# mims-harvard/ProCyon

Measured on AMD Instinct MI355X. Metric: phenotype-gen tokens/sec (ProCyon-Full greedy generation, end to end), higher is better.
Workload: dtype bf16; 1 GPU; configs[1]: ProCyon-Full (ESM2-650M + Llama-3-8B geometry=full) bf16 batch=1, 1024-residue protein, 512-token prompt, 256-token greedy generation; parallelism=single GPU

## Files before the change

include/pcy.h:

```cpp
#ifndef PCY_H
#define PCY_H
#include <stddef.h>
#include <stdint.h>

#ifdef __cplusplus
extern "C" {
#endif

#define PCY_ABI_VERSION 13

typedef struct pcy_ctx pcy_ctx;

enum { PCY_EPI_STORE = 0, PCY_EPI_RESID = 1, PCY_EPI_GELU_ERF = 2, PCY_EPI_GELU_ESM = 3, PCY_EPI_SWIGLU = 4 };
enum { PCY_POOL_MEAN = 0, PCY_POOL_MEAN_CORRECTED = 1, PCY_POOL_MAX = 2 };

int pcy_abi_version(void);
unsigned long long pcy_debug_dispatch_count(int kind);
unsigned long long pcy_debug_extend_grouped_count(void);
const char* pcy_last_error(void);
int pcy_ctx_create(int device_id, void* stream, pcy_ctx** out);
void pcy_ctx_destroy(pcy_ctx* ctx);
int pcy_ctx_sync(pcy_ctx* ctx);
int pcy_timer_start(pcy_ctx* ctx);
int pcy_timer_stop(pcy_ctx* ctx, float* ms_out);
// ... 156 lines not shown
int pcy_llama_decode_gemm_mq(pcy_ctx*, const pcy_llama_desc*, const pcy_kv_cache*, const pcy_gen_state*, int B);
unsigned long long pcy_debug_attn_mq_count(void);
int pcy_attn_decode_split(pcy_ctx*, void* qkv, int ld, const pcy_kv_cache* kv, int layer, void* o, int ldo, const int32_t* pos,
                          const void* cos_t, const void* sin_t, const uint8_t* keep, int B, int H, int Hkv, int dh);
int pcy_attn_split_chunk_keys(int B, int rows_per_prefix, int H, int Hkv, int dh, int prefix_T);
int pcy_llama_decode_split(pcy_ctx*, const pcy_llama_desc*, const pcy_kv_cache*, const pcy_gen_state*, int B);
int pcy_llama_decode_gemm_split(pcy_ctx*, const pcy_llama_desc*, const pcy_kv_cache*, const pcy_gen_state*, int B);
unsigned long long pcy_debug_attn_split_count(void);
int pcy_gemv_w8(pcy_ctx*, const void* W8, const float* scale, const void* x, int ldx, const void* resid, void* y, int ldy, const void* rms_w,
                float rms_eps, int rms_cast, int N, int K, int B, int epi);
int pcy_llama_decode_w8(pcy_ctx*, const pcy_llama_desc*, const pcy_llama_layer_fp8* w8, const pcy_kv_cache*, const pcy_gen_state*, int B);
int pcy_llama_greedy_w8(pcy_ctx*, const pcy_llama_desc*, const pcy_llama_layer_fp8* w8, const pcy_kv_cache*, const pcy_gen_state*, int B,
                        int n_steps, int use_graph);
unsigned long long pcy_debug_decode_w8_count(void);
int pcy_greedy_pick(pcy_ctx*, const pcy_llama_desc*, const pcy_kv_cache*, const pcy_gen_state*, int B, int advance_pos);
typedef struct {
  int32_t* hist;
  int32_t* n_hist;
  int32_t* window;
  const int32_t* forced;
  int32_t* counters;
  int32_t* last;
  int32_t cap, W;
  int32_t ngram_max, ngram_min;
} pcy_look_state;
int pcy_look_draft(pcy_ctx*, const pcy_llama_desc*, const pcy_look_state*, const pcy_gen_state*, void* embeds_out);
int pcy_look_verify(pcy_ctx*, const pcy_llama_desc*, const pcy_look_state*, const pcy_gen_state*, const void* logits);
unsigned long long pcy_debug_look_count(int which);
int pcy_attn_window(pcy_ctx*, void* qkv, int ld, const pcy_kv_cache* kv, int layer, void* o, int ldo, const int32_t* pos, const void* cos_t,
                    const void* sin_t, int W, int H, int Hkv, int dh);
// ... 97 lines not shown
```

procyon_amd/_lib.py:

```python
from __future__ import annotations

import ctypes as C
import os

_HERE = os.path.dirname(os.path.abspath(__file__))
LIB_PATH = os.environ.get("PCY_LIB") or os.path.join(_HERE, "libpcy.so")

EPI_STORE, EPI_RESID, EPI_GELU_ERF, EPI_GELU_ESM, EPI_SWIGLU = range(5)
POOL_MEAN, POOL_MEAN_CORRECTED, POOL_MAX = range(3)
ABI_VERSION = 13
(DISPATCH_GEMM_128, DISPATCH_GEMM_64, DISPATCH_GEMM_BIG, DISPATCH_GEMM_BIG_PERSIST, DISPATCH_GEMM_SPLITK, DISPATCH_GEMM_FP8, DISPATCH_ATTN_FAST,
 DISPATCH_DEC_STEP_GQA, DISPATCH_GEMM_MID, DISPATCH_ESM_GRAPH, DISPATCH_DEC_STEP_MHA, DISPATCH_DEC_LAYER, DISPATCH_DEC_STEP_NB, DISPATCH_DEC_STEP_MB,
 DISPATCH_DEC_LOOP_STREAM, DISPATCH_DEC_LOOP_MFMA, DISPATCH_SHARED_PREFIX, DISPATCH_XENT, DISPATCH_EXTEND,
 DISPATCH_EXTEND_PACKED) = range(20)
DISPATCH_DECODE = dict(step_gqa=DISPATCH_DEC_STEP_GQA, step_mha=DISPATCH_DEC_STEP_MHA, layer=DISPATCH_DEC_LAYER, step_nb=DISPATCH_DEC_STEP_NB,
                       step_mb=DISPATCH_DEC_STEP_MB, loop_stream=DISPATCH_DEC_LOOP_STREAM, loop_mfma=DISPATCH_DEC_LOOP_MFMA)
ATTN_ROUTE_DH32, ATTN_ROUTE_DH64, ATTN_ROUTE_LDS128_1, ATTN_ROUTE_LDS128_2 = range(4)

vp = C.c_void_p
i32 = C.c_int32
ci = C.c_int


class MlpDesc(C.Structure):
# ... 146 lines not shown
    "pcy_llama_decode_gemm": (ci, [vp, C.POINTER(LlamaDesc), C.POINTER(KvCache), C.POINTER(GenState), ci]),
    "pcy_debug_decode_gemm_count": (C.c_ulonglong, []),
    "pcy_attn_decode_shared": (ci, [vp, vp, ci, C.POINTER(KvCache), ci, vp, ci, vp, vp, vp, vp, ci, ci, ci, ci]),
    "pcy_llama_decode_gemm_mq": (ci, [vp, C.POINTER(LlamaDesc), C.POINTER(KvCache), C.POINTER(GenState), ci]),
    "pcy_debug_attn_mq_count": (C.c_ulonglong, []),
    "pcy_attn_decode_split": (ci, [vp, vp, ci, C.POINTER(KvCache), ci, vp, ci, vp, vp, vp, vp, ci, ci, ci, ci]),
    "pcy_attn_split_chunk_keys": (ci, [ci, ci, ci, ci, ci, ci]),
    "pcy_llama_decode_split": (ci, [vp, C.POINTER(LlamaDesc), C.POINTER(KvCache), C.POINTER(GenState), ci]),
    "pcy_llama_decode_gemm_split": (ci, [vp, C.POINTER(LlamaDesc), C.POINTER(KvCache), C.POINTER(GenState), ci]),
    "pcy_debug_attn_split_count": (C.c_ulonglong, []),
    "pcy_gemv_w8": (ci, [vp, vp, vp, vp, ci, vp, vp, ci, vp, C.c_float, ci, ci, ci, ci, ci]),
    "pcy_llama_decode_w8": (ci, [vp, C.POINTER(LlamaDesc), C.POINTER(LlamaLayerFp8), C.POINTER(KvCache), C.POINTER(GenState), ci]),
    "pcy_llama_greedy_w8": (ci, [vp, C.POINTER(LlamaDesc), C.POINTER(LlamaLayerFp8), C.POINTER(KvCache), C.POINTER(GenState), ci, ci, ci]),
    "pcy_debug_decode_w8_count": (C.c_ulonglong, []),
    "pcy_greedy_pick": (ci, [vp, C.POINTER(LlamaDesc), C.POINTER(KvCache), C.POINTER(GenState), ci, ci]),
    "pcy_look_draft": (ci, [vp, C.POINTER(LlamaDesc), C.POINTER(LookState), C.POINTER(GenState), vp]),
    "pcy_look_verify": (ci, [vp, C.POINTER(LlamaDesc), C.POINTER(LookState), C.POINTER(GenState), vp]),
    "pcy_debug_look_count": (C.c_ulonglong, [ci]),
    "pcy_attn_window": (ci, [vp, vp, ci, C.POINTER(KvCache), ci, vp, ci, vp, vp, vp, ci, ci, ci, ci]),
    "pcy_attn_window_chunk": (ci, []),
    "pcy_llama_decode_window": (ci, [vp, C.POINTER(LlamaDesc), C.POINTER(KvCache), C.POINTER(GenState), vp, ci, vp]),
    "pcy_debug_decode_window_count": (C.c_ulonglong, []),
    "pcy_llama_greedy": (ci, [vp, C.POINTER(LlamaDesc), C.POINTER(KvCache), C.POINTER(GenState), ci, ci, ci]),
    "pcy_sample_pick": (ci, [vp, C.POINTER(LlamaDesc), C.POINTER(KvCache), C.POINTER(GenState), ci, ci, C.c_float, C.c_float, vp, vp]),
    "pcy_llama_sample": (ci, [vp, C.POINTER(LlamaDesc), C.POINTER(KvCache), C.POINTER(GenState), ci, ci, C.c_float, C.c_float, vp]),
    "pcy_beam_step": (ci, [vp, vp, ci, ci, ci, ci, C.c_float, C.POINTER(BeamState)]),
    "pcy_kv_reorder": (ci, [vp, C.POINTER(LlamaDesc), C.POINTER(KvCache), vp, ci, ci]),
    "pcy_kv_reorder_range": (ci, [vp, C.POINTER(LlamaDesc), C.POINTER(KvCache), vp, ci, ci, ci]),
    "pcy_llama_beam_steps": (ci, [vp, C.POINTER(LlamaDesc), C.POINTER(KvCache), C.POINTER(GenState), ci, ci, ci, C.c_float, C.POINTER(BeamState), vp, ci, ci]),
    "pcy_llama_beam_steps_split": (ci, [vp, C.POINTER(LlamaDesc), C.POINTER(KvCache), C.POINTER(GenState), ci, ci, ci, C.c_float, C.POINTER(BeamState), vp, ci, ci]),
# ... 33 lines not shown
```

procyon_amd/csrc/pcy_elem.hip:

```cpp
#include "pcy_internal.h"
#include "pcy_pick.h"

namespace {

constexpr int NT = 256;

__global__ __launch_bounds__(NT) void rmsnorm_kernel(const bf16_t* __restrict__ x, const bf16_t* __restrict__ w,
                                                     bf16_t* __restrict__ y, int d, float eps, int cast) {
  __shared__ float red[NT / 64];
  const bf16_t* xr = x + (size_t)blockIdx.x * d;
  bf16_t* yr = y + (size_t)blockIdx.x * d;
  float ss = 0.f;
  for (int k = threadIdx.x * 8; k < d; k += NT * 8) {
    const uint4 v = *reinterpret_cast<const uint4*>(xr + k);
    const uint32_t u[4] = {v.x, v.y, v.z, v.w};
#pragma unroll
    for (int j = 0; j < 4; ++j) { float a = lo_bf(u[j]), b = hi_bf(u[j]); ss += a * a + b * b; }
  }
  ss = block_sum<NT>(ss, red);
  const float rstd = rsqrtf(ss / (float)d + eps);
  for (int k = threadIdx.x * 8; k < d; k += NT * 8) {
    const uint4 v = *reinterpret_cast<const uint4*>(xr + k);
    const uint4 g = *reinterpret_cast<const uint4*>(w + k);
    const uint32_t u[4] = {v.x, v.y, v.z, v.w}, gg[4] = {g.x, g.y, g.z, g.w};
// ... 347 lines not shown
    const float v = wsum[((size_t)p * POOL_CH + ch) * d + c];
    if (mode == 2) a = fmaxf(a, v);
    else { a += v; n += wcnt[((size_t)p * POOL_CH + ch) * d + c]; }
  }
  out[(size_t)p * d + c] = (mode == 2) ? f2bf(a) : f2bf(rbf(a) / (float)n);
}


__global__ __launch_bounds__(PICK_NT) void pick_stage1_kernel(const bf16_t* __restrict__ logits, int V, PickPartial* __restrict__ part) {
  __shared__ float redv[PICK_NT / 64];
  __shared__ int redi[PICK_NT / 64];
  __shared__ float red[PICK_NT / 64];
  const int b = blockIdx.y, c = blockIdx.x;
  const int chunk = (V + PICK_NB - 1) / PICK_NB;
  const int lo = c * chunk, hi = (lo + chunk) < V ? (lo + chunk) : V;
  const bf16_t* lg = logits + (size_t)b * V;
  float best = -INFINITY;
  int bi = 0x7fffffff;
  for (int i = lo + threadIdx.x; i < hi; i += PICK_NT) {
    const float v = bf2f(lg[i]);
    if (v > best || (v == best && i < bi)) { best = v; bi = i; }
  }
#pragma unroll
  for (int o = 32; o > 0; o >>= 1) {
    const float ov = __shfl_xor(best, o, 64);
    const int oi = __shfl_xor(bi, o, 64);
    if (ov > best || (ov == best && oi < bi)) { best = ov; bi = oi; }
  }
  const int w = threadIdx.x >> 6;
  if ((threadIdx.x & 63) == 0) { redv[w] = best; redi[w] = bi; }
  __syncthreads();
  best = redv[0]; bi = redi[0];
  for (int i = 1; i < PICK_NT / 64; ++i)
    if (redv[i] > best || (redv[i] == best && redi[i] < bi)) { best = redv[i]; bi = redi[i]; }
  float se = 0.f;
  for (int i = lo + threadIdx.x; i < hi; i += PICK_NT) se += expf(bf2f(lg[i]) - best);
  se = block_sum<PICK_NT>(se, red);
  if (threadIdx.x == 0) part[b * PICK_NB + c] = PickPartial{best, bi, best > -INFINITY ? se : 0.f, 0};
}

__global__ __launch_bounds__(256) void pick_stage2_kernel(const bf16_t* __restrict__ logits, int V, const PickPartial* __restrict__ part,
                                                          int32_t* __restrict__ next_tok, int32_t* __restrict__ tokens_out, int max_steps,
                                                          float* __restrict__ logprob, int32_t* __restrict__ step_dev, int32_t* __restrict__ pos_dev,
                                                          int advance_pos, int B) {
  const int l = threadIdx.x & 63;
  const int step = *step_dev;
  for (int b = threadIdx.x >> 6; b < B; b += 4) {
    float best, se;
    int bi;
    pick_merge_row(part[b * PICK_NB + l], best, bi, se);
    if (l == 0) {
      const float lsm = pick_logprob(logits + (size_t)b * V, bi, best, se);
      logprob[b] += lsm;
      next_tok[b] = bi;
      tokens_out[(size_t)b * max_steps + step] = bi;
    }
  }
  __syncthreads();
  if (threadIdx.x == 0) { if (advance_pos) *pos_dev += 1; *step_dev = step + 1; }
}

constexpr int SMP_NT = 1024;

__global__ __launch_bounds__(PICK_NT) void sample_stage1_kernel(const bf16_t* __restrict__ logits, int V, float temperature,
                                                                float4* __restrict__ part) {
  __shared__ float red[PICK_NT / 64];
  const int b = blockIdx.y, c = blockIdx.x;
  const int chunk = (V + PICK_NB - 1) / PICK_NB;
  const int lo = c * chunk, hi = (lo + chunk) < V ? (lo + chunk) : V;
  const bf16_t* lg = logits + (size_t)b * V;
  const bool scaled = temperature != 1.0f;
  float mr = -INFINITY, ms = -INFINITY;
  for (int i = lo + threadIdx.x; i < hi; i += PICK_NT) {
    const float v = bf2f(lg[i]);
// ... 863 lines not shown
  if (nprot <= 0) return;
  float* wsum = reinterpret_cast<float*>(ws);
  int* wcnt = reinterpret_cast<int*>(wsum + (size_t)nprot * POOL_CH * d);
  hipLaunchKernelGGL(pool_partial_kernel, dim3(nprot, (d + 511) / 512, POOL_CH), dim3(NT), 0, s, h, d, seg, rng, mode, wsum, wcnt);
  hipLaunchKernelGGL(pool_finish_kernel, dim3(nprot, (d + NT - 1) / NT), dim3(NT), 0, s, wsum, wcnt, d, mode, out);
}
void pcy_launch_pick_stage1(hipStream_t s, const bf16_t* logits, int rows, int V, void* partials) {
  if (rows > 0) hipLaunchKernelGGL(pick_stage1_kernel, dim3(PICK_NB, rows), dim3(PICK_NT), 0, s, logits, V, reinterpret_cast<PickPartial*>(partials));
}
void pcy_launch_greedy_pick(hipStream_t s, const bf16_t* logits, int B, int V, int32_t* next_tok, int32_t* tokens_out,
                            int max_steps, float* logprob, int32_t* pos_dev, int32_t* step_dev, int advance_pos, void* partials) {
  hipLaunchKernelGGL(pick_stage1_kernel, dim3(PICK_NB, B), dim3(PICK_NT), 0, s, logits, V, reinterpret_cast<PickPartial*>(partials));
  hipLaunchKernelGGL(pick_stage2_kernel, dim3(1), dim3(256), 0, s, logits, V, reinterpret_cast<const PickPartial*>(partials), next_tok,
                     tokens_out, max_steps, logprob, step_dev, pos_dev, advance_pos, B);
}
int pcy_sample_max_vocab() { return SMP_NT * SMP_KMAX; }
void pcy_launch_sample_step(hipStream_t s, const bf16_t* logits, int B, int V, float temperature, float nucleus_p, const float* uniforms,
                            unsigned* hist, bf16_t* probs_out, int32_t* next_tok, int32_t* tokens_out, int max_steps, float* logprob,
                            int32_t* pos_dev, int32_t* step_dev, int advance_pos, void* partials, bf16_t* pbits) {
  hipLaunchKernelGGL(sample_stage1_kernel, dim3(PICK_NB, B), dim3(PICK_NT), 0, s, logits, V, temperature, reinterpret_cast<float4*>(partials));
  hipLaunchKernelGGL(sample_probs_kernel, dim3(PICK_NB, B), dim3(PICK_NT), 0, s, logits, V, reinterpret_cast<const float4*>(partials), temperature,
                     nucleus_p > 0.f ? 1 : 0, hist, pbits);
  hipLaunchKernelGGL(sample_stage2_kernel, dim3(B), dim3(SMP_NT), 0, s, logits, V, reinterpret_cast<const float4*>(partials), temperature,
                     nucleus_p, uniforms, hist, probs_out, next_tok, tokens_out, max_steps, logprob, step_dev, B, pbits);
  hipLaunchKernelGGL(sample_advance_kernel, dim3(1), dim3(64), 0, s, pos_dev, step_dev, advance_pos);
}
void pcy_launch_copy_rows(hipStream_t s, const bf16_t* src, int lds_, bf16_t* dst, int ldd, const int32_t* rows, int nrows, int d) {
  if (nrows > 0) hipLaunchKernelGGL(copy_rows_kernel, dim3(nrows), dim3(NT), 0, s, src, lds_, dst, ldd, rows, d);
}
void pcy_launch_l2norm_rows(hipStream_t s, const bf16_t* x, bf16_t* y, int rows, int d, float eps) {
// ... 46 lines not shown
```

procyon_amd/csrc/pcy_engine.hip:

```cpp
#include <stdio.h>
#include <stdlib.h>
#include <stdarg.h>
#include <string.h>
#include <dlfcn.h>
#include <vector>

#include "../../include/pcy.h"
#include "pcy_internal.h"

namespace {

thread_local char g_err[512] = "";

int fail(int code, const char* fmt, ...) {
  va_list ap;
  va_start(ap, fmt);
  vsnprintf(g_err, sizeof(g_err), fmt, ap);
  va_end(ap);
  return code;
}

#define HIP_TRY(expr)                                                                       \
  do {                                                                                      \
    hipError_t e_ = (expr);                                                                 \
// ... 1 lines not shown
  } while (0)

inline size_t align_up(size_t v, size_t a) { return (v + a - 1) / a * a; }

inline bool kv_shared(const pcy_kv_cache* kv) { return kv->prefix_k != nullptr || kv->prefix_v != nullptr || kv->prefix_T != 0; }
inline int kv_cap(const pcy_kv_cache* kv) { return kv->Tmax + (kv_shared(kv) ? kv->prefix_T : 0); }
unsigned long long g_pcy_extend_grouped = 0;
unsigned long long g_pcy_look[2] = {0, 0};
unsigned long long g_pcy_decode_gemm = 0;
unsigned long long g_pcy_attn_mq = 0;
unsigned long long g_pcy_attn_split = 0;
unsigned long long g_pcy_decode_w8 = 0;
unsigned long long g_pcy_decode_window = 0;
unsigned long long g_pcy_f32_stream = 0;
unsigned long long g_pcy_f32_select[2] = {0, 0};

}

void pcy_set_error(const char* fmt, ...) {
  va_list ap;
  va_start(ap, fmt);
  vsnprintf(g_err, sizeof(g_err), fmt, ap);
  va_end(ap);
}

enum GraphKind {
  KIND_GREEDY = 0,
  KIND_DECODE = 1,
  KIND_BEAM = 2,
  KIND_GREEDY_W8 = 3,
// ... 42 lines not shown
  size_t mc_tags_words = 0;
  PcySwitches mc_tags_sw = {};
  uint64_t layers_fp = 0;
  PcyLayerWeightsDev* dev_layers = nullptr;
  uint32_t* nb_tags[9] = {};
  unsigned* nb_sync = nullptr;
  unsigned* mb_flags = nullptr;
  size_t mb_flags_words = 0;
  unsigned* mb_sync = nullptr;
  uint32_t* op_tags = nullptr;
  size_t op_tags_words = 0;
  unsigned* smp_hist = nullptr;
  int smp_hist_rows = 0;
  bf16_t* smp_pbits = nullptr;
  size_t smp_pbits_elems = 0;
  char* beam_ws = nullptr;
  size_t beam_ws_bytes = 0;

  struct GraphSlot { uint64_t key[16]; hipGraphExec_t exec; unsigned long long stamp; };
  static constexpr int N_GSLOTS = 8;
  GraphSlot gslots[N_GSLOTS] = {};
  unsigned long long gstamp = 0;
  void drop_gslots() {
    for (auto& g : gslots) {
      if (g.exec) hipGraphExecDestroy(g.exec);
      g = GraphSlot{};
    }
  }

  int reserve(size_t bytes) {
// ... 96 lines not shown
int ensure_sync_words(pcy_ctx* c) {
  if (!c->n_cu) {
    hipDeviceProp_t prop;
    HIP_TRY(hipGetDeviceProperties(&prop, c->device));
    c->n_cu = prop.multiProcessorCount;
  }
  if (!c->xwg_err) {
    HIP_TRY(hipHostMalloc(reinterpret_cast<void**>(&c->xwg_err), 64, hipHostMallocMapped | hipHostMallocCoherent));
    memset(c->xwg_err, 0, 64);
  }
  if (!c->ao_sync) {
    const size_t bytes = (size_t)(64 + 2 * AO_MAX_LAYERS * AO_FLAGS) * sizeof(unsigned);
    HIP_TRY(hipMalloc(reinterpret_cast<void**>(&c->ao_sync), bytes));
    HIP_TRY(hipMemset(c->ao_sync, 0, bytes));
  }
  return 0;
}
uint64_t fnv1a(uint64_t h, std::initializer_list<const void*> ptrs) {
  for (const void* p : ptrs) h = (h ^ (uint64_t)(uintptr_t)p) * 1099511628211ull;
  return h;
}
constexpr uint64_t FNV_BASIS = 1469598103934665603ull;
uint64_t layers_fingerprint(const pcy_llama_desc* m) {
  uint64_t h = fnv1a(FNV_BASIS, {m->layers});
  for (int l = 0; l < m->n_layers; ++l) {
    const pcy_llama_layer& L = m->layers[l];
    h = fnv1a(h, {L.ln1, L.wqkv, L.wo, L.ln2, L.wgu, L.wdown});
  }
  return h;
}
// ... 365 lines not shown
void enqueue_lm_head(const DecodeCx& cx, const DecodePlan& p, void* logits_out, int xn_ready, bool force_stream = false) {
  const pcy_llama_desc* m = cx.m;
  PcyGemvArgs h{};
  h.W = (const bf16_t*)m->lm_head; h.x = cx.x; h.y = (bf16_t*)logits_out; h.rms_w = (const bf16_t*)m->final_norm; h.rms_eps = m->rms_eps;
  h.rms_cast = m->rms_cast; h.N = m->vocab; h.K = m->d; h.B = cx.B; h.ldx = m->d; h.ldy = m->vocab; h.epi = EPI_STORE;
  if (p.batched_head && !(p.nb_on && cx.B <= 4)) {
    norm_if_needed(cx, true, m->final_norm, &xn_ready);
    h.x = cx.xn; h.rms_w = nullptr;
  } else {
    h.force_stream = p.nb_on || force_stream;
  }
  pcy_launch_gemv(cx.c->stream, h);
}

void enqueue_decode(pcy_ctx* c, const pcy_llama_desc* m, const pcy_kv_cache* kv, const pcy_gen_state* st, int B, const PcySwitches& sw, bool layers_only = false,
                    bool split = false) {
  hipStream_t s = c->stream;
  const int d = m->d, dh = m->head_dim;
  const DecodeCx cx = decode_cx(c, m, kv, st, B);
  DecodePlan p = plan_decode(c, m, kv, B, sw);
  if (split) { p.defer_qkv_finish = false; p.attn_o = false; }
  if (layers_only) {
    if (p.epoch_word) pcy_launch_bump(s, p.epoch_word);
    if (p.tag_word) pcy_launch_bump(s, p.tag_word);
  } else {
    pcy_launch_embed_tokens_dev(s, (const bf16_t*)m->embed, st->next_tok, cx.x, B, d, p.epoch_word, p.tag_word);
  }
  const size_t tag_stride = tag_words_per_layer(m);
  bool step_done = false;
  const bool try_layer = p.path == DEC_STEP_GQA || p.path == DEC_STEP_MHA || p.path == DEC_LAYERS;
  int xn_ready = 0;
  if (p.path == DEC_STEP_NB) {
    const PcyDecodeStepArgs sa = step_args(cx, c->nb_tags[B], pcy_decode_nb_tag_words(B), 2 * AO_FLAGS, pcy_decode_nb_line_words(B));
    step_done = pcy_launch_decode_step_nb(s, c->device, attn_args(cx, p, -1), block_args(cx, p.tag_word, mc_trace(sw)), mlp_args(cx, p.tag_word), sa, c->n_cu,
                                          c->ao_sync, B, sw.nb_ub);
    if (step_done) ++g_pcy_dispatch[PCY_DISPATCH_DEC_STEP_NB];
  } else if (p.path == DEC_STEP_GQA || p.path == DEC_STEP_MHA) {
    const PcyDecodeStepArgs sa = step_args(cx, c->mc_tags, tag_stride, AO_FLAGS, 32 * 256);
    step_done = pcy_launch_decode_step(s, attn_args(cx, p, -1), block_args(cx, p.tag_word, mc_trace(sw)), mlp_args(cx, p.tag_word), sa, c->n_cu,
                                       c->ao_sync);
// ... 37 lines not shown
    const int b = (int)(i / chunks), c = (int)(i % chunks);
    const bf16_t* src = logits + (size_t)b * V + c * 8;
    bf16_t* dst = all + (step * B + b) * ld + c * 8;
    if (vec && c * 8 + 8 <= V) {
      const uint32_t w0 = src[0] | ((uint32_t)src[1] << 16), w1 = src[2] | ((uint32_t)src[3] << 16);
      const uint32_t w2 = src[4] | ((uint32_t)src[5] << 16), w3 = src[6] | ((uint32_t)src[7] << 16);
      *reinterpret_cast<uint4*>(dst) = make_uint4(w0, w1, w2, w3);
    } else {
      for (int e = 0; e < 8 && c * 8 + e < V; ++e) dst[e] = src[e];
    }
  }
}
void enqueue_store_logits(hipStream_t s, const void* logits, void* all, int ld, const int32_t* step_dev, int B, int V) {
  if (all) hipLaunchKernelGGL(store_logits_kernel, dim3(B >= 8 ? 256 : 64), dim3(256), 0, s, (const bf16_t*)logits, (bf16_t*)all, step_dev, B, V, ld > 0 ? ld : V);
}
void enqueue_pick(pcy_ctx* c, const pcy_llama_desc* m, const pcy_gen_state* st, int B, int advance_pos, int Tmax) {
  enqueue_store_logits(c->stream, st->logits, st->logits_all, st->logits_all_ld, st->step, B, m->vocab);
  pcy_launch_greedy_pick(c->stream, (const bf16_t*)st->logits, B, m->vocab, st->next_tok, st->tokens_out, st->max_steps,
                         st->logprob, st->pos, st->step, advance_pos, carve_decode_ws(c->ws, m, B, Tmax).partials);
}

void enqueue_sample(pcy_ctx* c, const pcy_llama_desc* m, const pcy_gen_state* st, int B, int advance_pos, int Tmax, float temperature,
                    float nucleus_p, const float* uniforms, bf16_t* probs_out) {
  hipStream_t s = c->stream;
  if (nucleus_p > 0.f) temperature = 1.0f;
  enqueue_store_logits(s, st->logits, st->logits_all, st->logits_all_ld, st->step, B, m->vocab);
  void* partials = carve_decode_ws(c->ws, m, B, Tmax).partials;
  pcy_launch_sample_step(s, (const bf16_t*)st->logits, B, m->vocab, temperature, nucleus_p, uniforms, c->smp_hist, probs_out, st->next_tok,
                         st->tokens_out, st->max_steps, st->logprob, st->pos, st->step, advance_pos, partials, c->smp_pbits);
}
int ensure_sample_state(pcy_ctx* c, int B, int V) {
  if ((size_t)B * V > c->smp_pbits_elems) {
    if (c->smp_pbits) { HIP_TRY(hipStreamSynchronize(c->stream)); HIP_TRY(hipFree(c->smp_pbits)); c->smp_pbits = nullptr; c->smp_pbits_elems = 0; }
    HIP_TRY(hipMalloc(reinterpret_cast<void**>(&c->smp_pbits), (size_t)B * V * 2));
// ... 98 lines not shown
}
void pcy_ctx_destroy(pcy_ctx* c) {
  if (!c) return;
  hipStreamSynchronize(c->stream);
  c->drop_graph();
  c->drop_gslots();
  if (c->ws) hipFree(c->ws);
  if (c->xwg_err) hipHostFree(c->xwg_err);
  if (c->ao_sync) hipFree(c->ao_sync);
  if (c->mc_tags) hipFree(c->mc_tags);
  if (c->dev_layers) hipFree(c->dev_layers);
  for (auto& t : c->nb_tags) if (t) hipFree(t);
  if (c->nb_sync) hipFree(c->nb_sync);
  if (c->mb_flags) hipFree(c->mb_flags);
  if (c->mb_sync) hipFree(c->mb_sync);
  if (c->op_tags) hipFree(c->op_tags);
  if (c->beam_ws) hipFree(c->beam_ws);
  if (c->smp_hist) hipFree(c->smp_hist);
  if (c->smp_pbits) hipFree(c->smp_pbits);
  if (c->ev0) hipEventDestroy(c->ev0);
  if (c->ev1) hipEventDestroy(c->ev1);
  if (c->cap_stream) hipStreamDestroy(c->cap_stream);
  delete c;
}
int pcy_ctx_sync(pcy_ctx* c) {
  HIP_TRY(hipStreamSynchronize(c->stream));
  return take_sticky_error(c);
}
int pcy_timer_start(pcy_ctx* c) { HIP_TRY(hipEventRecord(c->ev0, c->stream)); return 0; }
int pcy_timer_stop(pcy_ctx* c, float* ms) {
// ... 915 lines not shown
  if (int r = decode_prologue(c, m, kv, st, B, "pcy_llama_decode", step_ws_bytes, &sw)) return r;
  enqueue_decode(c, m, kv, st, B, sw);
  return check_launch("pcy_llama_decode");
}

int pcy_llama_decode_layers(pcy_ctx* c, const pcy_llama_desc* m, const pcy_kv_cache* kv, const pcy_gen_state* st, int B, int reps) {
  PCY_STICKY(c);
  PcySwitches sw;
  if (int r = decode_prologue(c, m, kv, st, B, "pcy_llama_decode_layers", step_ws_bytes, &sw)) return r;
  return run_steps(c, reps, false, "pcy_llama_decode_layers", DecodeGraphKey{}, [&] { enqueue_decode(c, m, kv, st, B, sw, true); });
}

int pcy_greedy_pick(pcy_ctx* c, const pcy_llama_desc* m, const pcy_kv_cache* kv, const pcy_gen_state* st, int B, int advance_pos) {
  PCY_STICKY(c);
  if (int r = c->reserve(decode_ws_bytes(m, B, kv_cap(kv)))) return r;
  enqueue_pick(c, m, st, B, advance_pos, kv_cap(kv));
  return check_launch("pcy_greedy_pick");
}

static int look_args(const char* what, const pcy_look_state* ls, const pcy_gen_state* st, PcyLookArgs* a) {
  if (!ls || !st) return fail(1, "%s: state missing", what);
  if (ls->W < 2 || ls->W > 32) return fail(1, "%s: W=%d outside [2, 32]", what, ls->W);
  if (ls->ngram_min < 1 || ls->ngram_max < ls->ngram_min || ls->ngram_max > 16)
    return fail(1, "%s: n-gram range [%d, %d] (1 <= min <= max <= 16)", what, ls->ngram_min, ls->ngram_max);
  if (ls->cap < 1 || !ls->hist || !ls->n_hist || !ls->window || !ls->counters || !ls->last) return fail(1, "%s: history / window / counters missing", what);
  if (!st->pos || !st->step || !st->next_tok || !st->tokens_out || !st->logprob || st->max_steps < 1) return fail(1, "%s: generation state incomplete", what);
  *a = PcyLookArgs{ls->hist, ls->n_hist, ls->window, ls->forced, ls->counters, ls->last, ls->cap, ls->W, ls->ngram_max, ls->ngram_min,
                   st->pos, st->step, st->next_tok, st->tokens_out, st->logprob, st->max_steps};
  return 0;
}
int pcy_look_draft(pcy_ctx* c, const pcy_llama_desc* m, const pcy_look_state* ls, const pcy_gen_state* st, void* embeds_out) {
// ... 12 lines not shown
  if (int r = look_args("pcy_look_verify", ls, st, &a)) return r;
  if (!logits) return fail(1, "pcy_look_verify: logits is NULL");
  if (int r = c->reserve(pcy_look_verify_ws_bytes(a.W))) return r;
  pcy_launch_look_verify(c->stream, a, (const bf16_t*)logits, m->vocab, (bf16_t*)st->logits_all, st->logits_all_ld, c->ws);
  ++g_pcy_look[1];
  return check_launch("pcy_look_verify");
}
unsigned long long pcy_debug_look_count(int which) { return (which == 0 || which == 1) ? g_pcy_look[which] : 0; }


int pcy_llama_greedy(pcy_ctx* c, const pcy_llama_desc* m, const pcy_kv_cache* kv, const pcy_gen_state* st, int B, int n_steps,
                     int use_graph) {
  PCY_STICKY(c);
  PcySwitches sw;
  if (int r = decode_prologue(c, m, kv, st, B, "pcy_llama_greedy", step_ws_bytes, &sw)) return r;
  DecodeGraphKey key;
  decode_graph_key(key, c, m, kv, st, B, KIND_GREEDY, sw);
  key_record(key, st);
  return run_steps(c, n_steps, use_graph != 0, "pcy_llama_greedy", key, [&] {
    enqueue_decode(c, m, kv, st, B, sw);
    enqueue_pick(c, m, st, B, 1, kv_cap(kv));
  });
}

int pcy_llama_decode_graph(pcy_ctx* c, const pcy_llama_desc* m, const pcy_kv_cache* kv, const pcy_gen_state* st, int B) {
  PCY_STICKY(c);
  PcySwitches sw;
  if (int r = decode_prologue(c, m, kv, st, B, "pcy_llama_decode_graph", step_ws_bytes, &sw)) return r;
  DecodeGraphKey key;
  decode_graph_key(key, c, m, kv, st, B, KIND_DECODE, sw);
  key_record(key, st);
  return run_steps(c, 1, true, "pcy_llama_decode_graph", key, [&] { enqueue_decode(c, m, kv, st, B, sw); });
}


static void enqueue_decode_gemm(pcy_ctx* c, const pcy_llama_desc* m, const pcy_kv_cache* kv, const pcy_gen_state* st, int B, bool mq, bool split = false) {
// ... 83 lines not shown
  if (pcy_gemv_w8_rows_per_pass(d) < 1 || pcy_gemv_w8_rows_per_pass(F) < 1 || pcy_gemv_w8_rows_per_pass(H * dh) < 1)
    return fail(1, "%s: a row of x (d, ffn or H*dh elements) does not fit in LDS", what);
  return c->reserve(decode_ws_bytes(m, B, kv_cap(kv)));
}
int pcy_llama_decode_w8(pcy_ctx* c, const pcy_llama_desc* m, const pcy_llama_layer_fp8* w8, const pcy_kv_cache* kv, const pcy_gen_state* st, int B) {
  PCY_STICKY(c);
  if (int r = decode_w8_check(c, m, w8, kv, st, B, "pcy_llama_decode_w8")) return r;
  enqueue_decode_w8(c, m, w8, kv, st, B);
  return check_launch("pcy_llama_decode_w8");
}
int pcy_llama_greedy_w8(pcy_ctx* c, const pcy_llama_desc* m, const pcy_llama_layer_fp8* w8, const pcy_kv_cache* kv, const pcy_gen_state* st, int B,
                        int n_steps, int use_graph) {
  PCY_STICKY(c);
  if (int r = decode_w8_check(c, m, w8, kv, st, B, "pcy_llama_greedy_w8")) return r;
  if (!st->step || !st->tokens_out || !st->logprob) return fail(1, "pcy_llama_greedy_w8: generation state incomplete");
  DecodeGraphKey key;
  key_base(key, KIND_GREEDY_W8, B, m, kv, st, c, layers_fingerprint(m));
  key.keep = st->keep; key.w8 = w8; key.w8_fp = w8_fingerprint(m, w8);
  key_record(key, st);
  return run_steps(c, n_steps, use_graph != 0, "pcy_llama_greedy_w8", key, [&] {
    enqueue_decode_w8(c, m, w8, kv, st, B);
    enqueue_pick(c, m, st, B, 1, kv_cap(kv));
  });
}
unsigned long long pcy_debug_decode_w8_count(void) { return g_pcy_decode_w8; }

struct F32StreamCx { float *x, *xn, *qkv, *ao, *act; };
static F32StreamCx f32_stream_carve(char* ws, const pcy_f32_llama_desc* m, int B) {
  Carver cv(ws);
  F32StreamCx cx;
  cx.x = cv.take<float>((size_t)B * m->d);
  cx.xn = cv.take<float>((size_t)B * m->d);
  cx.qkv = cv.take<float>((size_t)B * (m->n_heads + 2 * m->n_kv_heads) * m->head_dim);
  cx.ao = cv.take<float>((size_t)B * m->n_heads * m->head_dim);
  cx.act = cv.take<float>((size_t)B * m->ffn);
  return cx;
}
static size_t f32_stream_ws_bytes(const pcy_f32_llama_desc* m, int B) {
  const size_t f = (size_t)B * (2 * (size_t)m->d + (size_t)(2 * m->n_heads + 2 * m->n_kv_heads) * m->head_dim + (size_t)m->ffn) * sizeof(float);
  return f + 8 * 256;
// ... 412 lines not shown
```

procyon_amd/csrc/pcy_internal.h:

```cpp
#pragma once
#include "pcy_common.h"
#include "pcy_switch.h"

struct PcyGemvArgs {
  const bf16_t* W;
  const bf16_t* x;
  bf16_t* y;
  const bf16_t* bias;
  const bf16_t* resid;
  const bf16_t* rms_w;
  float rms_eps;
  int rms_cast;
  int N, K, B, ldx, ldy, epi;
  int plain_loads;
  float* splitk_ws; size_t splitk_ws_bytes;
  const bf16_t* next_rms_w; bf16_t* next_xn; int* fused_next;
  int* defer_finish;
  int force_stream;
  int force_mfma;
  int krot;
};
void pcy_launch_gemv(hipStream_t s, const PcyGemvArgs& a);

struct PcyGemvW8Args {
// ... 317 lines not shown
  unsigned* err;
  unsigned long long* trace;
  int abl;
};
size_t pcy_decode_mb_flag_words();
int pcy_decode_mb_ds(int B);
bool pcy_decode_mb_fits(int B, int Tmax);
bool pcy_launch_decode_step_mb(hipStream_t s, int device, const PcyMbArgs& a, int n_cu);

size_t pcy_pool_ws_bytes(int nprot, int d);
void pcy_launch_pool(hipStream_t s, const bf16_t* h, int d, const int32_t* seg, const int32_t* rng, int nprot,
                     int mode, bf16_t* out, void* ws);
void pcy_launch_greedy_pick(hipStream_t s, const bf16_t* logits, int B, int V, int32_t* next_tok, int32_t* tokens_out,
                            int max_steps, float* logprob, int32_t* pos_dev, int32_t* step_dev, int advance_pos,
                            void* partials );
void pcy_launch_pick_stage1(hipStream_t s, const bf16_t* logits, int rows, int V, void* partials);
struct PcyLookArgs {
  int32_t* hist; int32_t* n_hist; int32_t* window; const int32_t* forced; int32_t* counters; int32_t* last;
  int cap, W, gmax, gmin;
  int32_t* pos; int32_t* step; int32_t* next_tok; int32_t* tokens_out; float* logprob; int max_steps;
};
size_t pcy_look_verify_ws_bytes(int W);
void pcy_launch_look_draft(hipStream_t s, const PcyLookArgs& a, const bf16_t* embed, int V, int d, bf16_t* embeds_out );
void pcy_launch_look_verify(hipStream_t s, const PcyLookArgs& a, const bf16_t* logits , int V, bf16_t* logits_all, int logits_all_ld,
                            void* partials );
void pcy_launch_retrieval_dot_f32(hipStream_t s, const float* query, int Q, const void* targets, int targets_bf16, int N, int D, float eps, float* sims);
size_t pcy_retrieval_dot_smem(int D);
void pcy_launch_retrieval_rank_f32(hipStream_t s, const float* sims, int Q, int N, int k, int32_t* idx_out, float* score_out);
int pcy_sample_max_vocab();
void pcy_launch_sample_step(hipStream_t s, const bf16_t* logits, int B, int V, float temperature, float nucleus_p, const float* uniforms,
// ... 26 lines not shown
```

procyon_amd/csrc/pcy_pick.h:

```cpp
#pragma once
#include "pcy_common.h"

constexpr int PICK_NT = 256;
constexpr int PICK_NB = 64;
struct PickPartial { float mx; int idx; float se; int pad; };

__device__ __forceinline__ void pick_merge_row(const PickPartial pp, float& best, int& bi, float& se) {
  best = pp.mx;
  bi = pp.idx;
#pragma unroll
  for (int o = 32; o > 0; o >>= 1) {
    const float ov = __shfl_xor(best, o, 64);
    const int oi = __shfl_xor(bi, o, 64);
    if (ov > best || (ov == best && oi < bi)) { best = ov; bi = oi; }
  }
  se = pp.se * expf(pp.mx - best);
  se = wave_sum(se);
}
__device__ __forceinline__ float pick_logprob(const bf16_t* __restrict__ row_logits, int bi, float best, float se) {
  return rbf((bf2f(row_logits[bi]) - best) - logf(se));
}
```

procyon_amd/csrc/pcy_switch.h:

```cpp
#pragma once
#include <stdint.h>
#include <stdlib.h>
#include <string.h>
#include <type_traits>

#define PCY_SWITCH_NAMES(X)                                                                                                                \
  X(attn_o) X(mlp_chain) X(decode_layer) X(decode_step) X(attn_qkv_finish) X(finish_norm) X(fp8_fused_norm) X(prefill_post_qkv) X(gemv_lds) \
  X(gemv_mfma4) X(fa_vrow) X(gelu_fast) X(esm_graph) X(lds_prefetch) X(decode_nb) X(decode_nb_step) X(beam_graph) X(kv_permute)             \
  X(decode_mb_step) X(beam_prefill_once) X(beam_kv_suffix) X(beam_kv_shared)
enum PcySwitch {
#define X(n) PCY_SW_##n,
  PCY_SWITCH_NAMES(X)
#undef X
  PCY_SW_COUNT
};
static_assert(PCY_SW_COUNT <= 32, "PcySwitches::off_mask holds one bit per name");

inline bool pcy_list_has(const char* list, const char* name) {
  if (!list) return false;
  const size_t n = strlen(name);
  for (const char* p = list; (p = strstr(p, name)) != nullptr; p += n)
    if ((p == list || p[-1] == ',') && (p[n] == 0 || p[n] == ',')) return true;
  return false;
}
// ... 39 lines not shown
```

Baseline: 397.1 tokens/s.

## Fuse logits store, greedy pick, and next-token embedding into one last-block kernel

Replaces the three-kernel greedy pick tail (store logits, stage-1 partials, stage-2 merge, plus the next step's embed kernel) with a single kernel. Each block copies its slice of logits and computes its partial. An atomic ticket elects the last block, which merges all partials, writes the token and logprob, bumps the step and pos counters, and gathers the next token's embedding row into the decode input buffer. The goal is to cut per-token kernel launches and the serialization gaps between them in the 256-step decode loop. In exchange it relies on a ticket counter with release/acquire fences, and it moves the first embed kernel out of the captured step.

```diff
diff --git a/include/pcy.h b/include/pcy.h
--- a/include/pcy.h
+++ b/include/pcy.h
@@ -194,6 +194,7 @@
                         int n_steps, int use_graph);
 unsigned long long pcy_debug_decode_w8_count(void);
 int pcy_greedy_pick(pcy_ctx*, const pcy_llama_desc*, const pcy_kv_cache*, const pcy_gen_state*, int B, int advance_pos);
+unsigned long long pcy_debug_pick_tail_count(int which);
 typedef struct {
   int32_t* hist;
   int32_t* n_hist;
diff --git a/procyon_amd/_lib.py b/procyon_amd/_lib.py
--- a/procyon_amd/_lib.py
+++ b/procyon_amd/_lib.py
@@ -184,6 +184,7 @@
     "pcy_llama_greedy_w8": (ci, [vp, C.POINTER(LlamaDesc), C.POINTER(LlamaLayerFp8), C.POINTER(KvCache), C.POINTER(GenState), ci, ci, ci]),
     "pcy_debug_decode_w8_count": (C.c_ulonglong, []),
     "pcy_greedy_pick": (ci, [vp, C.POINTER(LlamaDesc), C.POINTER(KvCache), C.POINTER(GenState), ci, ci]),
+    "pcy_debug_pick_tail_count": (C.c_ulonglong, [ci]),
     "pcy_look_draft": (ci, [vp, C.POINTER(LlamaDesc), C.POINTER(LookState), C.POINTER(GenState), vp]),
     "pcy_look_verify": (ci, [vp, C.POINTER(LlamaDesc), C.POINTER(LookState), C.POINTER(GenState), vp]),
     "pcy_debug_look_count": (C.c_ulonglong, [ci]),
diff --git a/procyon_amd/csrc/pcy_elem.hip b/procyon_amd/csrc/pcy_elem.hip
--- a/procyon_amd/csrc/pcy_elem.hip
+++ b/procyon_amd/csrc/pcy_elem.hip
@@ -385,29 +385,8 @@
   const int b = blockIdx.y, c = blockIdx.x;
   const int chunk = (V + PICK_NB - 1) / PICK_NB;
   const int lo = c * chunk, hi = (lo + chunk) < V ? (lo + chunk) : V;
-  const bf16_t* lg = logits + (size_t)b * V;
-  float best = -INFINITY;
-  int bi = 0x7fffffff;
-  for (int i = lo + threadIdx.x; i < hi; i += PICK_NT) {
-    const float v = bf2f(lg[i]);
-    if (v > best || (v == best && i < bi)) { best = v; bi = i; }
-  }
-#pragma unroll
-  for (int o = 32; o > 0; o >>= 1) {
-    const float ov = __shfl_xor(best, o, 64);
-    const int oi = __shfl_xor(bi, o, 64);
-    if (ov > best || (ov == best && oi < bi)) { best = ov; bi = oi; }
-  }
-  const int w = threadIdx.x >> 6;
-  if ((threadIdx.x & 63) == 0) { redv[w] = best; redi[w] = bi; }
-  __syncthreads();
-  best = redv[0]; bi = redi[0];
-  for (int i = 1; i < PICK_NT / 64; ++i)
-    if (redv[i] > best || (redv[i] == best && redi[i] < bi)) { best = redv[i]; bi = redi[i]; }
-  float se = 0.f;
-  for (int i = lo + threadIdx.x; i < hi; i += PICK_NT) se += expf(bf2f(lg[i]) - best);
-  se = block_sum<PICK_NT>(se, red);
-  if (threadIdx.x == 0) part[b * PICK_NB + c] = PickPartial{best, bi, best > -INFINITY ? se : 0.f, 0};
+  const PickPartial pp = pick_chunk_partial(logits + (size_t)b * V, lo, hi, redv, redi, red);
+  if (threadIdx.x == 0) part[b * PICK_NB + c] = pp;
 }
 
 __global__ __launch_bounds__(256) void pick_stage2_kernel(const bf16_t* __restrict__ logits, int V, const PickPartial* __restrict__ part,
@@ -429,6 +408,87 @@
   }
   __syncthreads();
   if (threadIdx.x == 0) { if (advance_pos) *pos_dev += 1; *step_dev = step + 1; }
+}
+
+__global__ __launch_bounds__(PICK_NT) void pick_tail_kernel(PcyPickTailArgs a) {
+  __shared__ float redv[PICK_NT / 64];
+  __shared__ int redi[PICK_NT / 64];
+  __shared__ float red[PICK_NT / 64];
+  __shared__ int last_s;
+  __shared__ int tok_s[PICK_EMBED_ROWS];
+  const int b = blockIdx.y, c = blockIdx.x, V = a.V, B = gridDim.y;
+  const int chunk = (V + PICK_NB - 1) / PICK_NB;
+  const int lo = c * chunk, hi = (lo + chunk) < V ? (lo + chunk) : V;
+  const bf16_t* lg = a.logits + (size_t)b * V;
+  PickPartial* part = reinterpret_cast<PickPartial*>(a.partials);
+  const int step = *a.step_dev;
+  if (a.all) {
+    const bool vec = (a.ld % 8 == 0) && ((reinterpret_cast<uintptr_t>(a.all) & 15) == 0);
+    bf16_t* row = a.all + ((size_t)step * B + b) * a.ld;
+    for (int p = ((lo + 7) >> 3) + threadIdx.x; p * 8 < hi; p += PICK_NT) {
+      const bf16_t* src = lg + p * 8;
+      bf16_t* dst = row + p * 8;
+      if (vec && p * 8 + 8 <= V) {
+        const uint32_t w0 = src[0] | ((uint32_t)src[1] << 16), w1 = src[2] | ((uint32_t)src[3] << 16);
+        const uint32_t w2 = src[4] | ((uint32_t)src[5] << 16), w3 = src[6] | ((uint32_t)src[7] << 16);
+        *reinterpret_cast<uint4*>(dst) = make_uint4(w0, w1, w2, w3);
+      } else {
+        for (int e = 0; e < 8 && p * 8 + e < V; ++e) dst[e] = src[e];
+      }
+    }
+  }
+  const PickPartial pp = pick_chunk_partial(lg, lo, hi, redv, redi, red);
+  if (threadIdx.x == 0) {
+    part[b * PICK_NB + c] = pp;
+    __builtin_amdgcn_fence(__ATOMIC_RELEASE, "agent");
+    asm volatile("s_waitcnt vmcnt(0)" ::: "memory");
+    const unsigned t = __hip_atomic_fetch_add(a.ticket, 1u, __ATOMIC_RELAXED, __HIP_MEMORY_SCOPE_AGENT);
+    const bool last = t == (unsigned)(PICK_NB * B) - 1u;
+    if (last) {
+      __builtin_amdgcn_fence(__ATOMIC_ACQUIRE, "agent");
+      asm volatile("s_waitcnt vmcnt(0)" ::: "memory");
+    }
+    last_s = last;
+  }
+  __syncthreads();
+  if (!last_s) return;
+  const int l = threadIdx.x & 63;
+  for (int r = threadIdx.x >> 6; r < B; r += PICK_NT / 64) {
+    float best, se;
+    int bi;
+    pick_merge_row(part[r * PICK_NB + l], best, bi, se);
+    if (l == 0) {
+      const float lsm = pick_logprob(a.logits + (size_t)r * V, bi, best, se);
+      a.logprob[r] += lsm;
+      a.next_tok[r] = bi;
+      a.tokens_out[(size_t)r * a.max_steps + step] = bi;
+      if (r < PICK_EMBED_ROWS) tok_s[r] = bi;
+    }
+  }
+  __syncthreads();
+  if (threadIdx.x == 0) {
+    if (a.advance_pos) *a.pos_dev += 1;
+    *a.step_dev = step + 1;
+    __hip_atomic_store(a.ticket, 0u, __ATOMIC_RELAXED, __HIP_MEMORY_SCOPE_AGENT);
+    if (a.table && a.epoch) *a.epoch += 1;
+    if (a.table && a.epoch2) *a.epoch2 += 1;
+  }
+  if (!a.table) return;
+  const int d8 = a.d >> 3, n = B * d8;
+  for (int i0 = threadIdx.x; i0 < n; i0 += PICK_NT * 8) {
+    uint4 v[8];
+#pragma unroll
+    for (int j = 0; j < 8; ++j) {
+      const int i = i0 + j * PICK_NT, r = i / d8, k = (i - r * d8) * 8;
+      v[j] = make_uint4(0, 0, 0, 0);
+      if (i < n) v[j] = *reinterpret_cast<const uint4*>(a.table + (size_t)tok_s[r] * a.d + k);
+    }
+#pragma unroll
+    for (int j = 0; j < 8; ++j) {
+      const int i = i0 + j * PICK_NT, r = i / d8, k = (i - r * d8) * 8;
+      if (i < n) *reinterpret_cast<uint4*>(a.x + (size_t)r * a.d + k) = v[j];
+    }
+  }
 }
 
 constexpr int SMP_NT = 1024;
@@ -1322,6 +1382,9 @@
   hipLaunchKernelGGL(pick_stage2_kernel, dim3(1), dim3(256), 0, s, logits, V, reinterpret_cast<const PickPartial*>(partials), next_tok,
                      tokens_out, max_steps, logprob, step_dev, pos_dev, advance_pos, B);
 }
+void pcy_launch_pick_tail(hipStream_t s, const PcyPickTailArgs& a, int B) {
+  hipLaunchKernelGGL(pick_tail_kernel, dim3(PICK_NB, B), dim3(PICK_NT), 0, s, a);
+}
 int pcy_sample_max_vocab() { return SMP_NT * SMP_KMAX; }
 void pcy_launch_sample_step(hipStream_t s, const bf16_t* logits, int B, int V, float temperature, float nucleus_p, const float* uniforms,
                             unsigned* hist, bf16_t* probs_out, int32_t* next_tok, int32_t* tokens_out, int max_steps, float* logprob,
diff --git a/procyon_amd/csrc/pcy_engine.hip b/procyon_amd/csrc/pcy_engine.hip
--- a/procyon_amd/csrc/pcy_engine.hip
+++ b/procyon_amd/csrc/pcy_engine.hip
@@ -39,6 +39,7 @@
 unsigned long long g_pcy_decode_window = 0;
 unsigned long long g_pcy_f32_stream = 0;
 unsigned long long g_pcy_f32_select[2] = {0, 0};
+unsigned long long g_pcy_pick_tail[2] = {0, 0};
 
 }
 
@@ -111,6 +112,7 @@
   int smp_hist_rows = 0;
   bf16_t* smp_pbits = nullptr;
   size_t smp_pbits_elems = 0;
+  unsigned* pick_ticket = nullptr;
   char* beam_ws = nullptr;
   size_t beam_ws_bytes = 0;
 
@@ -237,6 +239,12 @@
     HIP_TRY(hipMalloc(reinterpret_cast<void**>(&c->ao_sync), bytes));
     HIP_TRY(hipMemset(c->ao_sync, 0, bytes));
   }
+  return 0;
+}
+int ensure_pick_ticket(pcy_ctx* c) {
+  if (c->pick_ticket) return 0;
+  HIP_TRY(hipMalloc(reinterpret_cast<void**>(&c->pick_ticket), 64));
+  HIP_TRY(hipMemset(c->pick_ticket, 0, 64));
   return 0;
 }
 uint64_t fnv1a(uint64_t h, std::initializer_list<const void*> ptrs) {
@@ -632,7 +640,7 @@
 }
 
 void enqueue_decode(pcy_ctx* c, const pcy_llama_desc* m, const pcy_kv_cache* kv, const pcy_gen_state* st, int B, const PcySwitches& sw, bool layers_only = false,
-                    bool split = false) {
+                    bool split = false, bool embedded = false) {
   hipStream_t s = c->stream;
   const int d = m->d, dh = m->head_dim;
   const DecodeCx cx = decode_cx(c, m, kv, st, B);
@@ -641,7 +649,7 @@
   if (layers_only) {
     if (p.epoch_word) pcy_launch_bump(s, p.epoch_word);
     if (p.tag_word) pcy_launch_bump(s, p.tag_word);
-  } else {
+  } else if (!embedded) {
     pcy_launch_embed_tokens_dev(s, (const bf16_t*)m->embed, st->next_tok, cx.x, B, d, p.epoch_word, p.tag_word);
   }
   const size_t tag_stride = tag_words_per_layer(m);
@@ -709,10 +717,25 @@
 void enqueue_store_logits(hipStream_t s, const void* logits, void* all, int ld, const int32_t* step_dev, int B, int V) {
   if (all) hipLaunchKernelGGL(store_logits_kernel, dim3(B >= 8 ? 256 : 64), dim3(256), 0, s, (const bf16_t*)logits, (bf16_t*)all, step_dev, B, V, ld > 0 ? ld : V);
 }
-void enqueue_pick(pcy_ctx* c, const pcy_llama_desc* m, const pcy_gen_state* st, int B, int advance_pos, int Tmax) {
-  enqueue_store_logits(c->stream, st->logits, st->logits_all, st->logits_all_ld, st->step, B, m->vocab);
-  pcy_launch_greedy_pick(c->stream, (const bf16_t*)st->logits, B, m->vocab, st->next_tok, st->tokens_out, st->max_steps,
-                         st->logprob, st->pos, st->step, advance_pos, carve_decode_ws(c->ws, m, B, Tmax).partials);
+struct NextEmbed { bf16_t* x; unsigned* epoch_word; unsigned* tag_word; };
+void enqueue_pick(pcy_ctx* c, const pcy_llama_desc* m, const pcy_gen_state* st, int B, int advance_pos, int Tmax, const PcySwitches& sw,
+                  const NextEmbed* next = nullptr) {
+  void* partials = carve_decode_ws(c->ws, m, B, Tmax).partials;
+  if (sw.off(PCY_SW_pick_tail)) {
+    enqueue_store_logits(c->stream, st->logits, st->logits_all, st->logits_all_ld, st->step, B, m->vocab);
+    pcy_launch_greedy_pick(c->stream, (const bf16_t*)st->logits, B, m->vocab, st->next_tok, st->tokens_out, st->max_steps,
+                           st->logprob, st->pos, st->step, advance_pos, partials);
+    return;
+  }
+  PcyPickTailArgs a{};
+  a.logits = (const bf16_t*)st->logits; a.V = m->vocab; a.partials = partials;
+  a.all = (bf16_t*)st->logits_all; a.ld = st->logits_all_ld > 0 ? st->logits_all_ld : m->vocab;
+  a.next_tok = st->next_tok; a.tokens_out = st->tokens_out; a.max_steps = st->max_steps; a.logprob = st->logprob; a.pos_dev = st->pos; a.step_dev = st->step;
+  a.advance_pos = advance_pos; a.ticket = c->pick_ticket;
+  if (next) { a.table = (const bf16_t*)m->embed; a.x = next->x; a.d = m->d; a.epoch = next->epoch_word; a.epoch2 = next->tag_word; }
+  pcy_launch_pick_tail(c->stream, a, B);
+  ++g_pcy_pick_tail[0];
+  if (next) ++g_pcy_pick_tail[1];
 }
 
 void enqueue_sample(pcy_ctx* c, const pcy_llama_desc* m, const pcy_gen_state* st, int B, int advance_pos, int Tmax, float temperature,
@@ -841,6 +864,7 @@
   if (c->nb_sync) hipFree(c->nb_sync);
   if (c->mb_flags) hipFree(c->mb_flags);
   if (c->mb_sync) hipFree(c->mb_sync);
+  if (c->pick_ticket) hipFree(c->pick_ticket);
   if (c->op_tags) hipFree(c->op_tags);
   if (c->beam_ws) hipFree(c->beam_ws);
   if (c->smp_hist) hipFree(c->smp_hist);
@@ -1786,7 +1810,10 @@
 int pcy_greedy_pick(pcy_ctx* c, const pcy_llama_desc* m, const pcy_kv_cache* kv, const pcy_gen_state* st, int B, int advance_pos) {
   PCY_STICKY(c);
   if (int r = c->reserve(decode_ws_bytes(m, B, kv_cap(kv)))) return r;
-  enqueue_pick(c, m, st, B, advance_pos, kv_cap(kv));
+  const PcySwitches sw = pcy_read_switches();
+  if (!sw.off(PCY_SW_pick_tail))
+    if (int r = ensure_pick_ticket(c)) return r;
+  enqueue_pick(c, m, st, B, advance_pos, kv_cap(kv), sw);
   return check_launch("pcy_greedy_pick");
 }
 
@@ -1829,12 +1856,18 @@
   PCY_STICKY(c);
   PcySwitches sw;
   if (int r = decode_prologue(c, m, kv, st, B, "pcy_llama_greedy", step_ws_bytes, &sw)) return r;
+  if (!sw.off(PCY_SW_pick_tail))
+    if (int r = ensure_pick_ticket(c)) return r;
+  const bool tail = !sw.off(PCY_SW_pick_tail) && B <= PICK_EMBED_ROWS;
   DecodeGraphKey key;
   decode_graph_key(key, c, m, kv, st, B, KIND_GREEDY, sw);
   key_record(key, st);
+  const DecodePlan p = plan_decode(c, m, kv, B, sw);
+  const NextEmbed next{carve_decode_ws(c->ws, m, B, kv_cap(kv)).x, p.epoch_word, p.tag_word};
+  if (tail && n_steps > 0) pcy_launch_embed_tokens_dev(c->stream, (const bf16_t*)m->embed, st->next_tok, next.x, B, m->d, p.epoch_word, p.tag_word);
   return run_steps(c, n_steps, use_graph != 0, "pcy_llama_greedy", key, [&] {
-    enqueue_decode(c, m, kv, st, B, sw);
-    enqueue_pick(c, m, st, B, 1, kv_cap(kv));
+    enqueue_decode(c, m, kv, st, B, sw, false, false, tail);
+    enqueue_pick(c, m, st, B, 1, kv_cap(kv), sw, tail ? &next : nullptr);
   });
 }
 
@@ -1948,16 +1981,20 @@
   PCY_STICKY(c);
   if (int r = decode_w8_check(c, m, w8, kv, st, B, "pcy_llama_greedy_w8")) return r;
   if (!st->step || !st->tokens_out || !st->logprob) return fail(1, "pcy_llama_greedy_w8: generation state incomplete");
+  const PcySwitches sw = pcy_read_switches();
+  if (!sw.off(PCY_SW_pick_tail))
+    if (int r = ensure_pick_ticket(c)) return r;
   DecodeGraphKey key;
   key_base(key, KIND_GREEDY_W8, B, m, kv, st, c, layers_fingerprint(m));
-  key.keep = st->keep; key.w8 = w8; key.w8_fp = w8_fingerprint(m, w8);
+  key.sw = sw; key.keep = st->keep; key.w8 = w8; key.w8_fp = w8_fingerprint(m, w8);
   key_record(key, st);
   return run_steps(c, n_steps, use_graph != 0, "pcy_llama_greedy_w8", key, [&] {
     enqueue_decode_w8(c, m, w8, kv, st, B);
-    enqueue_pick(c, m, st, B, 1, kv_cap(kv));
+    enqueue_pick(c, m, st, B, 1, kv_cap(kv), sw);
   });
 }
 unsigned long long pcy_debug_decode_w8_count(void) { return g_pcy_decode_w8; }
+unsigned long long pcy_debug_pick_tail_count(int which) { return (which == 0 || which == 1) ? g_pcy_pick_tail[which] : 0; }
 
 struct F32StreamCx { float *x, *xn, *qkv, *ao, *act; };
 static F32StreamCx f32_stream_carve(char* ws, const pcy_f32_llama_desc* m, int B) {
diff --git a/procyon_amd/csrc/pcy_internal.h b/procyon_amd/csrc/pcy_internal.h
--- a/procyon_amd/csrc/pcy_internal.h
+++ b/procyon_amd/csrc/pcy_internal.h
@@ -355,6 +355,16 @@
 void pcy_launch_greedy_pick(hipStream_t s, const bf16_t* logits, int B, int V, int32_t* next_tok, int32_t* tokens_out,
                             int max_steps, float* logprob, int32_t* pos_dev, int32_t* step_dev, int advance_pos,
                             void* partials );
+constexpr int PICK_EMBED_ROWS = 8;
+struct PcyPickTailArgs {
+  const bf16_t* logits; int V;
+  void* partials;
+  bf16_t* all; int ld;
+  int32_t* next_tok; int32_t* tokens_out; int max_steps; float* logprob; int32_t* pos_dev; int32_t* step_dev; int advance_pos;
+  unsigned* ticket;
+  const bf16_t* table; bf16_t* x; int d; unsigned* epoch; unsigned* epoch2;
+};
+void pcy_launch_pick_tail(hipStream_t s, const PcyPickTailArgs& a, int B);
 void pcy_launch_pick_stage1(hipStream_t s, const bf16_t* logits, int rows, int V, void* partials);
 struct PcyLookArgs {
   int32_t* hist; int32_t* n_hist; int32_t* window; const int32_t* forced; int32_t* counters; int32_t* last;
diff --git a/procyon_amd/csrc/pcy_pick.h b/procyon_amd/csrc/pcy_pick.h
--- a/procyon_amd/csrc/pcy_pick.h
+++ b/procyon_amd/csrc/pcy_pick.h
@@ -4,6 +4,31 @@
 constexpr int PICK_NT = 256;
 constexpr int PICK_NB = 64;
 struct PickPartial { float mx; int idx; float se; int pad; };
+
+__device__ __forceinline__ PickPartial pick_chunk_partial(const bf16_t* __restrict__ lg, int lo, int hi, float* redv, int* redi, float* red) {
+  float best = -INFINITY;
+  int bi = 0x7fffffff;
+  for (int i = lo + threadIdx.x; i < hi; i += PICK_NT) {
+    const float v = bf2f(lg[i]);
+    if (v > best || (v == best && i < bi)) { best = v; bi = i; }
+  }
+#pragma unroll
+  for (int o = 32; o > 0; o >>= 1) {
+    const float ov = __shfl_xor(best, o, 64);
+    const int oi = __shfl_xor(bi, o, 64);
+    if (ov > best || (ov == best && oi < bi)) { best = ov; bi = oi; }
+  }
+  const int w = threadIdx.x >> 6;
+  if ((threadIdx.x & 63) == 0) { redv[w] = best; redi[w] = bi; }
+  __syncthreads();
+  best = redv[0]; bi = redi[0];
+  for (int i = 1; i < PICK_NT / 64; ++i)
+    if (redv[i] > best || (redv[i] == best && redi[i] < bi)) { best = redv[i]; bi = redi[i]; }
+  float se = 0.f;
+  for (int i = lo + threadIdx.x; i < hi; i += PICK_NT) se += expf(bf2f(lg[i]) - best);
+  se = block_sum<PICK_NT>(se, red);
+  return PickPartial{best, bi, best > -INFINITY ? se : 0.f, 0};
+}
 
 __device__ __forceinline__ void pick_merge_row(const PickPartial pp, float& best, int& bi, float& se) {
   best = pp.mx;
diff --git a/procyon_amd/csrc/pcy_switch.h b/procyon_amd/csrc/pcy_switch.h
--- a/procyon_amd/csrc/pcy_switch.h
+++ b/procyon_amd/csrc/pcy_switch.h
@@ -7,7 +7,7 @@
 #define PCY_SWITCH_NAMES(X)                                                                                                                \
   X(attn_o) X(mlp_chain) X(decode_layer) X(decode_step) X(attn_qkv_finish) X(finish_norm) X(fp8_fused_norm) X(prefill_post_qkv) X(gemv_lds) \
   X(gemv_mfma4) X(fa_vrow) X(gelu_fast) X(esm_graph) X(lds_prefetch) X(decode_nb) X(decode_nb_step) X(beam_graph) X(kv_permute)             \
-  X(decode_mb_step) X(beam_prefill_once) X(beam_kv_suffix) X(beam_kv_shared)
+  X(decode_mb_step) X(beam_prefill_once) X(beam_kv_suffix) X(beam_kv_shared) X(pick_tail)
 enum PcySwitch {
 #define X(n) PCY_SW_##n,
   PCY_SWITCH_NAMES(X)
```

After: 398.2 tokens/s, median of 6. About the same (+0.3%).
